# google/deepvariant

Hardware: AMD Instinct MI355X
Metric: candidate pileups/sec (encode+CNN) (higher is better)
Workload: dtype u8 (encoder) / f16 MFMA, f32 accumulate (CNN); 1 GPU; configs[1] shape: synthetic 30x Illumina pileups, WGS 100x221x7, HIP encode + Inception-v3 MFMA on 1 MI355X per rank, random-init weights; parallelism=interval shards x1, all-gather of probs, collective_world_size=1

## Files before the change

deepvariant_amd/csrc/model.hip:

```cpp
#include <algorithm>
#include <map>
#include <atomic>
#include <cmath>
#include <cstdlib>
#include <cstring>
#include <memory>
#include <thread>

#include <hip/hip_fp16.h>

#include "model_graph.h"
#include "model_kernels.h"
#include "block35.h"
#include "mixed3.h"
#include "chain.h"
#include "stem_fused.h"
#include "calib.h"
#include "layer_export.h"

namespace {

static int stem_sub_batch() {
  static const int v = getenv("DV_STEM_SB") ? std::max(1, atoi(getenv("DV_STEM_SB"))) : (1 << 30);
  return v;
// ... 50 lines not shown
  if (mode >= 2) return true;
  return m->blank_conv4_op >= 0 && &op == &m->ops[m->blank_conv4_op];
}

struct Pass {
  dv_model* m;
  int n;
  hipStream_t stream;
  int first, last;
  int shifted_buf, out_example_off;
  size_t images_off;
  std::vector<char> side_pooled;
  _Float16* out_ptr(int buf) const {
    const size_t halfs = static_cast<size_t>(out_example_off) * m->buffers[buf].bytes_per_example() / 2;
    return m->buf_ptr(buf) + (buf == shifted_buf ? halfs : 0);
  }
};

dv::C8Geom c8_geom(const BufferDesc& b) {
  const TensorGeom g = b.geom();
  return dv::C8Geom{g.h, g.w, g.halo, g.hp, g.wp, g.groups};
}


int enqueue_stem_a(const Pass& ps, int oi) {
  const dv_model* m = ps.m;
  const int n = ps.n;
  const Op &op = m->ops[oi], &c2 = m->ops[oi + 1];
  dv::StemAArgs a{};
  a.in = nullptr;
  a.in_ind = &ext_table(m)->images;
  a.in_off = ps.images_off;
  a.w1 = m->w_ptr(op);
  a.w2 = m->w_ptr(c2);
  a.shift1 = m->shift_ptr(op);
  a.shift2 = m->shift_ptr(c2);
  a.out = m->buf_ptr(c2.out_buf);
  a.og = c8_geom(m->buffers[c2.out_buf]);
  a.N = n;
  a.H = op.ih;
  a.W = op.iw;
  a.C = op.cin_real;
  a.OH1 = op.oh;
  a.OW1 = op.ow;
  a.OH2 = c2.oh;
  a.OW2 = c2.ow;
  a.tiles_y = (c2.oh + dv::kStemA_TH - 1) / dv::kStemA_TH;
  a.tiles_x = (c2.ow + dv::kStemA_TW - 1) / dv::kStemA_TW;
  a.total_tiles = n * a.tiles_y * a.tiles_x;
  a.in_bytes = static_cast<unsigned>(static_cast<size_t>(n) * op.ih * op.iw * op.cin_real);
  if (m->blank_on()) {
    a.blank_thr = m->blank_thr(1);
    a.blank_src = static_cast<const _Float16*>(m->d_blank_c2.ptr);
    a.blank_need = m->blank_thr(5);
  }
  TraceScope tr(ps.stream, std::string(m->blank_on() ? "[blank tiles copied] " : "") + "stem_a conv3x3s2 " + std::to_string(op.cin_real) + "->32 + conv3x3 32->32 (fused)",
                2.0 * n * (static_cast<double>(op.oh) * op.ow * op.kh * op.kw * op.cin_real * op.cout +
                           static_cast<double>(c2.oh) * c2.ow * 9 * 32 * 32),
                static_cast<double>(n) * (op.ih * op.iw * op.cin_real + 2.0 * c2.oh * c2.ow * 32));
  dv::ProfileScope prof(dv::kProfConv, ps.stream);
  dv::launch_stem_a(a, m->stem_a_grid, ps.stream);
  return 2;
}

void report_stem_b_profile(dv::StemBArgs a, int grid, hipStream_t stream) {
  const size_t words = static_cast<size_t>(grid) * 16;
  unsigned long long* d = nullptr;
  if (hipMalloc(&d, words * 8) != hipSuccess) return;
  (void)hipMemsetAsync(d, 0, words * 8, stream);
  a.prof = d;
  dv::launch_stem_b(a, grid, stream);
  std::vector<unsigned long long> h(words);
  (void)hipStreamSynchronize(stream);
  (void)hipMemcpy(h.data(), d, words * 8, hipMemcpyDeviceToHost);
  (void)hipFree(d);
  for (int w = 0; w < 2; ++w) {
    double sum[7] = {0, 0, 0, 0, 0, 0, 0};
    for (int b = 0; b < grid; ++b)
      for (int i = 0; i < 7; ++i) sum[i] += static_cast<double>(h[(b * 2 + w) * 8 + i]);
    const double tiles = static_cast<double>(a.total_tiles);
    fprintf(stderr, "[dv-stem-b wave %d] cycles/tile: issue %.0f conv3 %.0f dma-wait %.0f barrierA %.0f pool %.0f "
                    "barrierB %.0f conv1x1+store %.0f\n", w ? 7 : 0, sum[0] / tiles, sum[1] / tiles,
            sum[6] / tiles, sum[2] / tiles, sum[3] / tiles, sum[4] / tiles, sum[5] / tiles);
  }
  std::map<unsigned long long, std::vector<int>> where;
  for (int b = 0; b < grid; ++b) {
    const unsigned long long v = h[(b * 2) * 8 + 7];
    const unsigned hw = static_cast<unsigned>(v), xcc = static_cast<unsigned>(v >> 32);
    where[(static_cast<unsigned long long>(xcc) << 16) | ((hw >> 8) & 0xffu)].push_back(b);
  }
  int pairs = 0, same_parity = 0, apart256 = 0;
  for (const auto& kv : where) {
    if (kv.second.size() != 2) continue;
    ++pairs;
    const unsigned t0 = (static_cast<unsigned>(h[(kv.second[0] * 2) * 8 + 7]) >> 16) & 15u;
    const unsigned t1 = (static_cast<unsigned>(h[(kv.second[1] * 2) * 8 + 7]) >> 16) & 15u;
    same_parity += (t0 & 1u) == (t1 & 1u);
    apart256 += kv.second[1] - kv.second[0] == 256;
  }
  fprintf(stderr, "[dv-stem-b placement] %zu places for %d workgroups; %d pairs, %d with TG slots of EQUAL parity, "
                  "%d pairs are blocks b / b+256\n", where.size(), grid, pairs, same_parity, apart256);
  for (int cls = 0; cls < 2; ++cls) {
    double sum[7] = {0, 0, 0, 0, 0, 0, 0};
    int nb = 0;
    for (int b = 0; b < grid; ++b) {
      const unsigned tg = (static_cast<unsigned>(h[(b * 2) * 8 + 7]) >> 16) & 15u;
      if (static_cast<int>(tg & 1u) != cls) continue;
      ++nb;
      for (int i = 0; i < 7; ++i) sum[i] += static_cast<double>(h[(b * 2) * 8 + i]);
    }
    double tot = 0;
    for (double v : sum) tot += v;
    fprintf(stderr, "[dv-stem-b TG parity %d] %d workgroups, share of wave-0 cycles: issue %.3f conv3 %.3f dma-wait %.3f "
                    "barrierA %.3f pool %.3f barrierB %.3f conv1x1+store %.3f; cycles per workgroup %.0f\n", cls, nb,
            sum[0] / tot, sum[1] / tot, sum[6] / tot, sum[2] / tot, sum[3] / tot, sum[4] / tot, sum[5] / tot,
            nb ? tot / nb : 0.0);
  }
}

int enqueue_stem_b(const Pass& ps, int oi) {
  const dv_model* m = ps.m;
  const int n = ps.n;
  const Op &op = m->ops[oi], &c4 = m->ops[oi + 1];
  const BufferDesc& ib = m->buffers[op.in_buf];
  dv::StemBArgs a{};
  a.in = m->buf_ptr(op.in_buf);
  a.w3 = m->w_ptr(op);
  a.w4 = m->w_ptr(c4);
  a.shift3 = m->shift_ptr(op);
  a.shift4 = m->shift_ptr(c4);
  a.out = m->buf_ptr(c4.out_buf);
  a.ig = c8_geom(ib);
  a.og = c8_geom(m->buffers[c4.out_buf]);
  a.N = n;
  a.OH3 = op.oh;
  a.OW3 = op.ow;
  a.PH = c4.oh;
  a.PW = c4.ow;
  a.Cout4 = c4.cout;
  a.tiles_y = (c4.oh + dv::kStemB_PH - 1) / dv::kStemB_PH;
  a.tiles_x = (c4.ow + dv::kStemB_PW - 1) / dv::kStemB_PW;
  a.total_tiles = n * a.tiles_y * a.tiles_x;
  a.in_bytes = static_cast<size_t>(n) * ib.bytes_per_example();
  a.in_img_bytes = static_cast<unsigned>(ib.bytes_per_example());
  if (m->blank_on()) {
    a.blank_thr = m->blank_thr(2);
    a.blank_src = static_cast<const _Float16*>(m->d_blank_b.ptr);
    a.blank_need = m->blank_thr(6);
  }
  TraceScope tr(ps.stream, std::string(m->blank_on() ? "[blank tiles copied] " : "") + "stem_b conv3x3 32->64 + maxpool3s2 + conv1x1 64->" + std::to_string(c4.cout) + " (fused)",
                2.0 * n * (static_cast<double>(op.oh) * op.ow * 9 * 32 * 64 +
                           static_cast<double>(c4.oh) * c4.ow * 64 * c4.cout),
                2.0 * n * (static_cast<double>(op.ih) * op.iw * 32 + static_cast<double>(c4.oh) * c4.ow * c4.cout));
  dv::ProfileScope prof(dv::kProfConv, ps.stream);
  static const bool stem_prof = getenv("DV_STEM_PROF") != nullptr;
  if (stem_prof && g_trace != nullptr) {
    report_stem_b_profile(a, m->stem_b_grid, ps.stream);
  } else {
    dv::launch_stem_b(a, m->stem_b_grid, ps.stream);
  }
  return 2;
}

int enqueue_block35(const Pass& ps, int oi) {
  const dv_model* m = ps.m;
  const int n = ps.n;
  const Op &op = m->ops[oi], &r5 = m->ops[oi + 1], &r3 = m->ops[oi + 2], &pj = m->ops[oi + 3];
  const Op &c5 = m->ops[oi + 4], &c3a = m->ops[oi + 5], &c3b = m->ops[oi + 6], &ap = m->ops[oi + 7];
  const BufferDesc& ib = m->buffers[op.in_buf];
  dv::Block35Args a{};
  a.in = m->buf_ptr(op.in_buf);
  a.ig = ib.geom();
  a.in_img_bytes = static_cast<unsigned>(ib.bytes_per_example());
  a.N = n;
  a.h = op.oh;
  a.w = op.ow;
  a.n_chunks = op.cin / kChunk;
  a.w1 = m->w_ptr(op);
  a.sh_red5 = m->shift_ptr(r5);
  a.sh_red3 = m->shift_ptr(r3);
  a.sh_b1 = m->shift_ptr(op);
  a.sh_pool = m->shift_ptr(ap);
  a.pool_c = pj.cout;
  a.w5 = m->w_ptr(c5);
  a.sh5 = m->shift_ptr(c5);
  a.w3a = m->w_ptr(c3a);
  a.sh3a = m->shift_ptr(c3a);
  a.w3b = m->w_ptr(c3b);
  a.sh3b = m->shift_ptr(c3b);
  a.out = m->buf_ptr(op.out_buf);
  a.og = m->buffers[op.out_buf].geom();
  a.goff_b1 = op.out_coff / 8;
  a.goff_5 = c5.out_coff / 8;
  a.goff_3 = c3b.out_coff / 8;
  a.goff_pool = ap.out_coff / 8;
  const double px = static_cast<double>(n) * op.oh * op.ow;
  const double tr_flops = 2.0 * px * (static_cast<double>(op.cin) * (op.cout + r5.cout + r3.cout + pj.cout) +
                                      25.0 * c5.cin * c5.cout + 9.0 * c3a.cin * c3a.cout + 9.0 * c3b.cin * c3b.cout);
  const std::string tr_label = "block35 " + std::to_string(op.cin) + "->" + std::to_string(op.cout) + "|" +
                               std::to_string(r5.cout) + "->" + std::to_string(c5.cout) + " 5x5|" +
                               std::to_string(r3.cout) + "->" + std::to_string(c3a.cout) + "->" +
                               std::to_string(c3b.cout) + " 3x3|" + std::to_string(pj.cout) + " pool @" +
                               std::to_string(op.oh) + "x" + std::to_string(op.ow);
// ... 389 lines not shown
    return dv::fail(DV_ERR_INVALID_ARGUMENT,
                    "dv_model_create: unsupported shape (need H,W >= 75, C <= 16, max_batch <= 8192)");
  }
  int n_dev = 0;
  if (hipGetDeviceCount(&n_dev) != hipSuccess || n_dev <= 0) {
    return dv::fail(DV_ERR_NO_DEVICE, "no HIP device: libdvhip has no CPU fallback");
  }
  if (device < 0 || device >= n_dev) {
    return dv::fail(DV_ERR_INVALID_ARGUMENT, "bad device ordinal");
  }
  DV_HIP_CHECK(hipSetDevice(device));
  std::unique_ptr<dv_model> m(new dv_model());
  m->device = device;
  m->desc = *desc;
  m->precise = getenv("DV_PRECISE") != nullptr ? atoi(getenv("DV_PRECISE")) != 0 : desc->channels > 8;
  m->build();
  m->stem_a_grid = dv::stem_a_blocks(device);
  m->stem_b_grid = dv::stem_b_blocks(device);
  m->n_cus = dv::stem_a_blocks(device) / 2;
  for (const Op& op : m->ops) {
    const BufferDesc& ob = m->buffers[op.out_buf];
    const double pieces = static_cast<double>(desc->max_batch) * ob.bytes_per_example() / 16.0;
    const double pixels = static_cast<double>(desc->max_batch) * op.oh * op.ow;
    if (pieces >= 2147483648.0 || pixels >= 67108864.0) {
      return dv::fail(DV_ERR_INVALID_ARGUMENT,
                      "dv_model_create: max_batch too large for this image size (N*OH*OW must stay "
                      "below 2^26 and every activation tensor below 2^31 16-byte pieces)");
    }
  }
  if (static_cast<double>(desc->max_batch) * desc->height * desc->width * desc->channels >=
      2147483648.0) {
    return dv::fail(DV_ERR_INVALID_ARGUMENT, "dv_model_create: max_batch * H * W * C must be < 2^31");
  }
  m->dbuf.resize(m->buffers.size());
  for (size_t i = 0; i < m->buffers.size(); ++i) {
    const BufferDesc& b = m->buffers[i];
    const bool stem_buf = static_cast<int>(i) < m->stem_out_buf;
    const size_t examples = std::max(
        static_cast<size_t>(stem_buf ? std::min(desc->max_batch, stem_sub_batch()) : desc->max_batch),
        static_cast<size_t>(b.min_examples));
    const size_t bytes = examples * b.bytes_per_example() +
                         static_cast<size_t>(8) * (b.h + 2 * b.halo) * (b.w + 2 * b.halo) * 16;
    if (int rc = m->dbuf[i].reserve(bytes)) return rc;
    DV_HIP_CHECK(hipMemset(m->dbuf[i].ptr, 0, m->dbuf[i].cap));
  }
  if (int rc = m->d_w.reserve(m->packed_halfs * 2)) return rc;
  if (int rc = m->d_shift.reserve(m->shift_floats * 4)) return rc;
  if (int rc = m->d_dense_w.reserve(static_cast<size_t>(m->feat_c) * desc->num_classes * 4)) return rc;
  if (int rc = m->d_dense_b.reserve(desc->num_classes * 4)) return rc;
  if (int rc = m->d_ext.reserve(sizeof(ExtPtrs))) return rc;
  if (!(getenv("DV_BLANK_SKIP") != nullptr && atoi(getenv("DV_BLANK_SKIP")) == 0) &&
      m->ops[0].first_u8 && m->blank_conv4_op >= 0 && m->ops[m->blank_conv4_op].group_followers == 0 &&
      (static_cast<size_t>(desc->height) * desc->width * desc->channels) % 4 == 0) {
    if (int rc = m->d_blank_thr.reserve(static_cast<size_t>(7) * desc->max_batch * sizeof(int))) return rc;
    DV_HIP_CHECK(hipMemset(m->d_blank_thr.ptr, 0, m->d_blank_thr.cap));
    m->blank_skip = true;
  }
  *out = m.release();
  return DV_OK;
}

void dv_model_destroy(dv_model* m) {
  if (!m) return;
  (void)hipSetDevice(m->device);
  for (auto& b : m->dbuf) b.release();
  m->d_w.release();
  m->d_shift.release();
  m->d_dense_w.release();
  m->d_dense_b.release();
  m->d_tbl.release();
  m->d_blank_thr.release();
  m->d_ext.release();
  m->d_blank_conv4.release();
  m->d_blank_c2.release();
  m->d_blank_b.release();
  for (auto& g : m->graphs) (void)hipGraphExecDestroy(g.exec);
  delete m;
}

int64_t dv_model_num_params(const dv_model* m) { return m ? m->n_params : 0; }

int64_t dv_model_conv_macs(const dv_model* m) {
  if (!m) return 0;
  int64_t macs = 0;
  for (const Op& op : m->ops) {
    if (op.type == kOpConv) {
      macs += static_cast<int64_t>(op.kh) * op.kw * op.cin_real * op.cout * op.oh * op.ow;
    }
  }
  return macs;
}

int dv_model_num_layers(const dv_model* m) {
  return m ? static_cast<int>(m->layers.size()) : 0;
}

int dv_model_layer_info(const dv_model* m, int layer, int32_t* kh, int32_t* kw,
                        int32_t* cin, int32_t* cout, int64_t* param_offset) {
  if (!m || layer < 0 || layer >= static_cast<int>(m->layers.size())) {
    return dv::fail(DV_ERR_INVALID_ARGUMENT, "dv_model_layer_info: bad layer");
  }
  const LayerInfo& l = m->layers[layer];
  if (kh) *kh = l.kh;
  if (kw) *kw = l.kw;
  if (cin) *cin = l.cin;
  if (cout) *cout = l.cout;
  if (param_offset) *param_offset = l.param_off;
  return DV_OK;
}
// ... 675 lines not shown
```

deepvariant_amd/csrc/model_graph.h:

```cpp
#ifndef DV_MODEL_GRAPH_H_
#define DV_MODEL_GRAPH_H_

#include <string>
#include <vector>

#include "dv_internal.h"
#include "conv_mfma.h"
#include "imgconv.h"

namespace dv {
namespace graph {

using namespace convk;

struct TensorRef {
  int buf = -1;
  int h = 0, w = 0, c = 0;
};

struct BufferDesc {
  int h, w, c;
  int halo = 0;
  int min_examples = 1;
  bool f32 = false;
// ... 28 lines not shown
  bool pool_shift_relu = false;
  bool pool_in = false;
  int side_pool_partner = -1;
  int avg_partner = -1;
  int avg_tile_g = 0;
  bool pool_out = false;
  int band = 0;
  bool split = false;
  bool split_rows = false;
  int split_tiles = 0;
  bool v2 = false;
  int v2_g = 0;
  int v2_steps = 0;
  int v2_tiles = 0;
  bool stem_a = false;
  bool stem_b = false;
  int chain_len = 0;
  int chain_g = 0;
  int chain_tpx = 0;
  bool in_chain = false;
  int b35 = 0;
  int m3 = 0;
};

struct LayerInfo {
  int kh, kw, cin, cout;
  int64_t param_off;
};

}
}

using namespace dv::graph;

struct dv_model {
  int device = 0;
  dv_model_desc desc{};
  std::vector<BufferDesc> buffers;
  std::vector<Op> ops;
  std::vector<LayerInfo> layers;
  int64_t n_params = 0;
  int feat_buf = -1, feat_p = 0, feat_c = 0;
  int stem_ops_end = 0, stem_out_buf = -1;
  int stem_a_grid = 512, stem_b_grid = 256;
  int n_cus = 256;
  size_t packed_halfs = 0, shift_floats = 0, tbl_entries = 0;
  std::vector<dv::DeviceBuffer> dbuf;
  dv::DeviceBuffer d_w, d_shift, d_dense_w, d_dense_b, d_tbl;
  bool blank_skip = false;
  bool blank_enabled = true;
  bool blank_ready = false;
  int blank_conv4_op = -1;
  dv::DeviceBuffer d_blank_thr;
  dv::DeviceBuffer d_blank_conv4;
  dv::DeviceBuffer d_blank_c2;
  dv::DeviceBuffer d_blank_b;
  bool blank_on() const { return blank_ready && blank_enabled; }
  bool precise = false;
  bool wide_stage = false;
  bool loaded = false;
  std::vector<float> h_shift, h_dense_b;
  dv::DeviceBuffer d_ext;
  struct GraphEntry {
    int n;
    hipStream_t stream;
    hipGraphExec_t exec;
  };
  std::vector<GraphEntry> graphs;
  int64_t graph_captures = 0, graph_replays = 0;
  struct NamedView {
    std::string name;
    int buf, coff, c;
  };
  std::vector<NamedView> named_views;

  template <typename T = _Float16>
  T* buf_ptr(int buf) const { return static_cast<T*>(dbuf[buf].ptr); }
  const _Float16* w_ptr(const Op& op) const { return static_cast<const _Float16*>(d_w.ptr) + op.w_off; }
  const float* shift_ptr(const Op& op) const { return static_cast<const float*>(d_shift.ptr) + op.shift_off; }
  const int* blank_thr(int row) const { return static_cast<const int*>(d_blank_thr.ptr) + row * desc.max_batch; }

  int new_buffer(int h, int w, int c);
  static int pick_nb(int cout);
  TensorRef conv(TensorRef x, int cout, int kh, int kw, int stride = 1, bool same = true,
                 int dst_buf = -1, int dst_coff = 0, int cin_real = -1);
  TensorRef full(int buf) const;
  void pooled_projection(TensorRef x, int cout, int dst_buf, int dst_coff);
  TensorRef pool(OpType type, TensorRef x, int dst_buf = -1, int dst_coff = 0);
  void group_siblings();
  dv::ImgConvArgs imgconv_geometry(const Op& op, int g) const;
  void choose_imgconv();
  void choose_band();
  void choose_side_pool();
  void choose_split();
  void choose_avg_epilogue();
  void choose_chains();
  void choose_block35();
  void choose_mixed3();
  void build();
  std::vector<size_t> correction_shift_offsets() const;
};

#endif
```

deepvariant_amd/csrc/model_kernels.hip:

```cpp
#include <cstdlib>

#include "model_kernels.h"
#include "stem_fused.h"

using namespace dv::convk;

namespace {

constexpr int kFirstUnroll = 5;

__global__ void set_ext_kernel(ExtPtrs* ext, const uint8_t* images, float* probs, const int32_t* rows_hint, int rows_add) {
  ext->images = images;
  ext->probs = probs;
  ext->rows_hint = rows_hint;
  ext->rows_add = rows_add;
}

__device__ __forceinline__ const uint8_t* ext_images(const ExtPtrs* ext, size_t off) {
  const unsigned long long v = reinterpret_cast<unsigned long long>(ext->images + off);
  const unsigned lo = __builtin_amdgcn_readfirstlane(static_cast<unsigned>(v));
  const unsigned up = __builtin_amdgcn_readfirstlane(static_cast<unsigned>(v >> 32));
  return reinterpret_cast<const uint8_t*>((static_cast<unsigned long long>(up) << 32) | lo);
}

// ... 114 lines not shown
                             co + 2 * hq + 1 < p.Cout ? p.shift[co + 2 * hq + 1] : 0.f};
        const float2_t v = float2_t{acc[pt][4 * q + 2 * hq], acc[pt][4 * q + 2 * hq + 1]} + sv;
        half2_t h = __builtin_convertvector(v, half2_t);
        h = __builtin_elementwise_max(h, zero2);
        pk[q][hq] = __builtin_bit_cast(unsigned, h);
      }
    }
#pragma unroll
    for (int t2 = 0; t2 < 2; ++t2) {
      const auto d0 = __builtin_amdgcn_permlane32_swap(pk[2 * t2][0], pk[2 * t2 + 1][0], false, false);
      const auto d1 = __builtin_amdgcn_permlane32_swap(pk[2 * t2][1], pk[2 * t2 + 1][1], false, false);
      const uint4_t piece = {d0[0], d1[0], d0[1], d1[1]};
      const int group = 2 * t2 + hi;
      if (mvalid[pt] && group * 8 < p.Cout) {
        outp[obase[pt] + static_cast<unsigned>(group) * gstride] = piece;
      }
    }
  }
}

__global__ void preprocess_kernel(const ExtPtrs* ext, size_t in_off, _Float16* out, size_t n_pix, int C,
                                  int H, int W, TensorGeom og) {
  const size_t i = blockIdx.x * static_cast<size_t>(blockDim.x) + threadIdx.x;
  if (i >= n_pix) return;
  const uint8_t* in = ext->images + in_off;
  const uint8_t* px = in + i * C;
  _Float16 v[16];
#pragma unroll
  for (int c = 0; c < 16; ++c) {
    v[c] = c < C ? static_cast<_Float16>((static_cast<float>(px[c]) - 128.0f) / 128.0f)
                 : static_cast<_Float16>(0.f);
  }
  const size_t n = i / (static_cast<size_t>(H) * W);
  const int pix = static_cast<int>(i - n * (static_cast<size_t>(H) * W));
  const int y = pix / W, x = pix - y * W;
  uint4* dst = reinterpret_cast<uint4*>(out);
  const size_t plane = static_cast<size_t>(og.hp) * og.wp;
  const size_t at = (n * 2) * plane + static_cast<size_t>(y + og.halo) * og.wp + x + og.halo;
  dst[at] = *reinterpret_cast<uint4*>(&v[0]);
  dst[at + plane] = *reinterpret_cast<uint4*>(&v[8]);
}

__global__ void blank_need_kernel(int* thr, int stride, int n, int oh2, int ph_b, int ow4, int p4, int stem_b_fused,
                                  int conv4_walks) {
  const int i = blockIdx.x * blockDim.x + threadIdx.x;
  if (i >= n) return;
  const int t4 = min(thr[2 * stride + i], ph_b);
  const int kb = (t4 + dv::kStemB_PH - 1) / dv::kStemB_PH;
  thr[5 * stride + i] = !stem_b_fused ? oh2 : kb > 0 ? min(oh2, 2 * dv::kStemB_PH * kb + 2) : 0;
  const int span = 31 / max(ow4, 1) + 1;
  int m5 = 0;
  for (int j = max(0, i - span); j <= min(n - 1, i + span); ++j) m5 = max(m5, min(thr[4 * stride + j], p4));
  thr[6 * stride + i] = !conv4_walks ? ph_b : m5 > 0 ? min(ph_b, 2 * m5 + 3) : 0;
}

__global__ __launch_bounds__(256) void blank_rows_kernel(const ExtPtrs* ext, size_t in_off, int n_hint0, int H,
                                                         int row_bytes, int* thr, int stride) {
  __shared__ int last;
  const uint8_t* images = ext->images + in_off;
  const int n = blockIdx.x, tid = threadIdx.x;
  const unsigned img_bytes = static_cast<unsigned>(H) * row_bytes;
  const uint32_t* img = reinterpret_cast<const uint32_t*>(images + static_cast<size_t>(n) * img_bytes);
  const int n_dw = static_cast<int>(img_bytes / 4);
  if (tid == 0) last = -1;
  __syncthreads();
  constexpr int kPer = 16;
  const bool hinted = ext->rows_hint != nullptr;
  const int hinted_rows = hinted ? max(0, min(H, ext->rows_hint[n_hint0 + n] + ext->rows_add)) : 0;
  for (int hi = hinted ? 0 : n_dw; hi > 0; hi -= 256 * kPer) {
    uint32_t v[kPer];
#pragma unroll
    for (int k = 0; k < kPer; ++k) {
      const int i = hi - 1 - (k * 256 + tid);
      v[k] = i >= 0 ? img[i] : 0u;
    }
    int mine = -1;
#pragma unroll
    for (int k = 0; k < kPer; ++k) {
      const int i = hi - 1 - (k * 256 + tid);
      if (v[k] != 0) mine = max(mine, 4 * i + 3 - (__clz(v[k]) >> 3));
    }
    if (mine >= 0) atomicMax(&last, mine);
    __syncthreads();
    if (last >= 0) break;
  }
  if (tid == 0) {
    const int r = hinted ? hinted_rows : last < 0 ? 0 : last / row_bytes + 1;
    const int t2 = (r + 1) / 2, t3 = t2 + 1, t4 = (t3 + 1) / 2;
    thr[n] = r;
    thr[stride + n] = t2;
    thr[2 * stride + n] = t4;
    thr[3 * stride + n] = t4;
    thr[4 * stride + n] = (t4 + 1) / 2;
  }
}

__global__ void maxpool3s2_kernel(PoolArgs p) {
  const int cg = p.C / 8;
  const size_t total = static_cast<size_t>(p.N) * cg * p.OH * p.OW;
  const size_t i = blockIdx.x * static_cast<size_t>(blockDim.x) + threadIdx.x;
  if (i >= total) return;
  const int ow = i % p.OW;
  size_t t = i / p.OW;
  const int oh = t % p.OH;
  t /= p.OH;
  const int g = t % cg;
  const int n = t / cg;
  const size_t plane = static_cast<size_t>(p.ig.hp) * p.ig.wp;
  const half8_t* src = reinterpret_cast<const half8_t*>(p.in) + (static_cast<size_t>(n) * p.ig.groups + g) * plane;
  const half8_t* src_lo = src + static_cast<size_t>(p.lo_in_groups) * plane;
  half8_t best, best_lo;
#pragma unroll
  for (int j = 0; j < 8; ++j) {
    best[j] = static_cast<_Float16>(-65504.f);
    best_lo[j] = static_cast<_Float16>(0.f);
  }
  const size_t at0 = static_cast<size_t>(oh * 2 + p.ig.halo) * p.ig.wp + ow * 2 + p.ig.halo;
  if (p.lo_in_groups > 0) {
    half8_t v[9], l[9];
#pragma unroll
    for (int t9 = 0; t9 < 9; ++t9) {
      const size_t at = at0 + static_cast<size_t>(t9 / 3) * p.ig.wp + t9 % 3;
      v[t9] = src[at];
      l[t9] = src_lo[at];
    }
#pragma unroll
    for (int t9 = 0; t9 < 9; ++t9) {
#pragma unroll
      for (int j = 0; j < 8; ++j) {
        const bool take = v[t9][j] > best[j] || (v[t9][j] == best[j] && l[t9][j] > best_lo[j]);
        best[j] = take ? v[t9][j] : best[j];
        best_lo[j] = take ? l[t9][j] : best_lo[j];
      }
    }
  } else {
    for (int dh = 0; dh < 3; ++dh)
      for (int dw = 0; dw < 3; ++dw) {
// ... 207 lines not shown
```

deepvariant_amd/csrc/stem.hip:

```cpp
#include <algorithm>
#include <type_traits>

#include "stem_fused.h"

namespace dv {
namespace {

typedef _Float16 half8_t __attribute__((ext_vector_type(8)));
typedef _Float16 half2_t __attribute__((ext_vector_type(2)));
typedef float float16_t __attribute__((ext_vector_type(16)));
typedef float float4_t __attribute__((ext_vector_type(4)));
typedef float float2_t __attribute__((ext_vector_type(2)));
typedef unsigned uint4_t __attribute__((ext_vector_type(4)));
typedef unsigned uint3_t __attribute__((ext_vector_type(3)));

__device__ __forceinline__ half8_t lds_piece(const char* smem, unsigned off) {
  return *reinterpret_cast<const half8_t*>(smem + off);
}

__device__ __forceinline__ float16_t acc_init(const float* tbl) {
  const float4_t* t = reinterpret_cast<const float4_t*>(tbl);
  const float4_t a = t[0], b = t[1], c = t[2], d = t[3];
  return float16_t{a[0], a[1], a[2], a[3], b[0], b[1], b[2], b[3],
                   c[0], c[1], c[2], c[3], d[0], d[1], d[2], d[3]};
// ... 210 lines not shown
    }
  };

  auto convert_patch = [&](unsigned org) {
#pragma unroll
    for (int ps = 0; ps < A_PASSES; ++ps) {
      if (sact && (ps * A_ROWS_PER_PASS + srow < A_INH)) {
        const unsigned a = org + srel + ps * spass;
        const unsigned s8 = (a & 3u) * 8u;
        const unsigned lo = __builtin_amdgcn_alignbit(pre[ps][1], pre[ps][0], s8);
        const unsigned up = __builtin_amdgcn_alignbit(pre[ps][2], pre[ps][1], s8);
        if constexpr (WIDE) {
          typedef unsigned uint2_t __attribute__((ext_vector_type(2)));
          const unsigned lo1 = __builtin_amdgcn_alignbit(pre[ps][3], pre[ps][2], s8);
          char* d = smem + sdst + ps * (A_ROWS_PER_PASS * AW_ROW);
          *reinterpret_cast<uint2_t*>(d) = uint2_t{lo, up};
          *reinterpret_cast<uint2_t*>(d + AW_PLANE) = uint2_t{lo1, 0u};
        } else {
          *reinterpret_cast<uint4_t*>(smem + sdst + ps * (A_ROWS_PER_PASS * A_INROW)) =
              normalise8(lo, up);
        }
      }
    }
  };
  auto copy_blank_tile = [&](int nb_, int yb, int xb) {
    const uint4_t* src = reinterpret_cast<const uint4_t*>(p.blank_src);
    uint4_t* dst = reinterpret_cast<uint4_t*>(p.out) + static_cast<size_t>(nb_) * img_out;
    const int th = min(A_TH, p.OH2 - yb), tw = min(A_TW, p.OW2 - xb);
    const int per_group = th * tw;
    constexpr int kPer = (4 * A_TH * A_TW + A_THREADS - 1) / A_THREADS;
    uint4_t v[kPer];
    unsigned at[kPer];
#pragma unroll
    for (int k = 0; k < kPer; ++k) {
      const int e = k * A_THREADS + tid;
      const int g = e / per_group, r = e - g * per_group;
      const int yy = r / tw, xx = r - yy * tw;
      at[k] = e < 4 * per_group ? static_cast<unsigned>(g) * gstride +
                                      static_cast<unsigned>((yb + yy + p.og.halo) * p.og.wp + xb + xx + p.og.halo)
                                : 0xffffffffu;
      if (at[k] != 0xffffffffu) v[k] = src[at[k]];
    }
#pragma unroll
    for (int k = 0; k < kPer; ++k) {
      if (at[k] != 0xffffffffu) dst[at[k]] = v[k];
    }
  };
  auto next_tile = [&](int tt) {
    if (p.blank_thr == nullptr) return tt;
    while (tt < p.total_tiles) {
      int nb_, yb, xb;
      tile_origin(tt, nb_, yb, xb);
      if (yb < p.blank_thr[nb_]) break;
      if (yb < p.blank_need[nb_]) copy_blank_tile(nb_, yb, xb);
      tt += gridDim.x;
    }
    return tt;
  };
  int t = next_tile(blockIdx.x);
  int n, y0, x0;
  unsigned origin = 0;
  if (t < p.total_tiles) {
    origin = tile_origin(t, n, y0, x0);
    issue_loads(origin);
    convert_patch(origin);
  }
  while (t < p.total_tiles) {
    __syncthreads();

#pragma unroll
    for (int round = 0; round < 2; ++round) {
      float16_t acc[2];
#pragma unroll
      for (int f = 0; f < 2; ++f) acc[f] = acc_init(lsh + hi * 16);
      if constexpr (WIDE) {
        typedef unsigned uint2_t __attribute__((ext_vector_type(2)));
        auto b_addr = [&](int tap, int f) {
          const int kh = tap / 3, kw = tap % 3;
          return bA[round * 2 + f] + static_cast<unsigned>((kw & 1) * 2 * AW_PLANE + kh * AW_ROW + (kw >> 1) * 8);
        };
        const char* w1l = smem + AW_OFF_W1 + (hi * 32 + l31) * 16;
        half8_t wa[2];
        uint2_t xb[2][2];
        wa[0] = lds_piece(w1l, 0);
#pragma unroll
        for (int f = 0; f < 2; ++f) xb[0][f] = *reinterpret_cast<const uint2_t*>(smem + b_addr(0, f));
#pragma unroll
        for (int tap = 0; tap < 9; ++tap) {
          if (tap + 1 < 9) {
            wa[(tap + 1) & 1] = lds_piece(w1l, (tap + 1) * 2 * 32 * 16);
#pragma unroll
            for (int f = 0; f < 2; ++f) xb[(tap + 1) & 1][f] = *reinterpret_cast<const uint2_t*>(smem + b_addr(tap + 1, f));
          }
#pragma unroll
          for (int f = 0; f < 2; ++f) {
            const half8_t x = __builtin_bit_cast(half8_t, normalise8(xb[tap & 1][f][0], xb[tap & 1][f][1]));
            acc[f] = __builtin_amdgcn_mfma_f32_32x32x16_f16(wa[tap & 1], x, acc[f], 0, 0, 0);
          }
        }
      } else
      mfma_sweep<5, 2, 3>(
          a1, smem,
          [&](int s, int f) {
            const int ff = round * 2 + f;
            return s < 3 ? bA[ff] + s * A_INROW : s == 3 ? bB[ff] + 16 : bC[ff] + 2 * A_INROW + 16;
          },
          acc);
// ... 56 lines not shown
constexpr int B_PTH = B_C3H + 2, B_PTW = B_C3W + 2;
constexpr int B_PTPX = B_PTH * B_PTW;
constexpr int B_PTPLANE = B_PTPX * 16;
constexpr int B_PT_BYTES = (4 * B_PTPLANE + 1023) / 1024 * 1024;
constexpr int B_PT_PIECES = 4 * B_PTPX;
constexpr int B_PPX = B_PH * B_PW;
constexpr int B_PFR = (B_PPX + 31) / 32;
constexpr int B_PPLANE = B_PFR * 32 * 16;
constexpr int B_THREADS = B_WAVES * 64;
constexpr int B_PASSES = (B_PT_PIECES + B_THREADS - 1) / B_THREADS;
constexpr int B_POOL_ROUNDS = (8 * B_PPX + B_THREADS - 1) / B_THREADS;
constexpr int B_OFF_C3 = 2 * B_PT_BYTES;
constexpr int B_OFF_P = (B_OFF_C3 + 8 * B_C3PLANE + 15) / 16 * 16;
constexpr int B_OFF_SH = B_OFF_P + 8 * B_PPLANE;
constexpr int B_LDS = B_OFF_SH + (64 + 96) * 4;
constexpr int B_BLOCKS_PER_CU = B_WAVES == 4 ? 2 : 1;
static_assert(B_LDS * B_BLOCKS_PER_CU <= 160 * 1024, "workgroups per CU");
static_assert(2 * B_PFR == B_WAVES, "1x1 work split: (pooled fragment, subtiles {0,1}) and (fragment, subtile 2)");
static_assert(B_C3FR <= 2 * B_WAVES, "two conv3 fragments per wave");

__global__ __launch_bounds__(B_THREADS, 2) void stem_b_kernel(StemBArgs p) {
  extern __shared__ __attribute__((aligned(16))) char smem[];
  const int tid = threadIdx.x;
  const int lane = tid & 63, wave = tid >> 6;
  const int hi = lane >> 5, l31 = lane & 31;
  const int wave_u = __builtin_amdgcn_readfirstlane(wave);

  half8_t a3lo[18], a3up[18];
#pragma unroll
  for (int kc = 0; kc < 18; ++kc) {
    a3lo[kc] = *reinterpret_cast<const half8_t*>(p.w3 + (((0 * 18 + kc) * 2 + hi) * 32 + l31) * 8);
    a3up[kc] = *reinterpret_cast<const half8_t*>(p.w3 + (((1 * 18 + kc) * 2 + hi) * 32 + l31) * 8);
  }
  const int s0 = wave < B_PFR ? 0 : 2;
  const int nsub = wave < B_PFR ? 2 : 1;
#pragma unroll
  for (int kc = 0; kc < 18; ++kc) {
    asm volatile("" : "+v"(a3lo[kc]));
    asm volatile("" : "+v"(a3up[kc]));
  }
  float* lsh = reinterpret_cast<float*>(smem + B_OFF_SH);
  if (tid < 160) {
    const int r = tid & 15, h = (tid >> 4) & 1;
    const int co = (r & 3) + 8 * (r >> 2) + 4 * h;
    if (tid < 64) {
      lsh[tid] = p.shift3[(tid >> 5) * 32 + co];
    } else {
      const int c4 = ((tid - 64) >> 5) * 32 + co;
      lsh[tid] = c4 < p.Cout4 ? p.shift4[c4] : 0.f;
    }
  }

  unsigned prel[B_PASSES];
#pragma unroll
  for (int ps = 0; ps < B_PASSES; ++ps) {
    const int e = ps * B_THREADS + tid;
    const int g = e / B_PTPX, rem = e - g * B_PTPX;
    const int row = rem / B_PTW, col = rem - row * B_PTW;
    prel[ps] = e < B_PT_PIECES
                   ? static_cast<unsigned>(((g * p.ig.hp + row) * p.ig.wp + col) * 16)
                   : 0x80000000u;
  }
  unsigned b3[2], c3dst[2];
  bool c3ok[2];
#pragma unroll
  for (int m = 0; m < 2; ++m) {
    const int i = (wave + B_WAVES * m) * 32 + l31;
    c3ok[m] = i < B_C3PX;
    const int ii = min(i, B_C3PX - 1);
    const int cy = ii / B_C3W, cx = ii - cy * B_C3W;
    b3[m] = static_cast<unsigned>(hi * B_PTPLANE + (cy * B_PTW + cx) * 16);
    c3dst[m] = static_cast<unsigned>(B_OFF_C3 + hi * B_C3PLANE + i * 16);
  }
  const int pp = (wave % B_PFR) * 32 + l31;
  const int ppc = min(pp, B_PPX - 1);
  const int ppy = ppc / B_PW, ppx = ppc - ppy * B_PW;
  const unsigned b4 = static_cast<unsigned>(B_OFF_P + hi * B_PPLANE + pp * 16);

  const int tiles_img = p.tiles_y * p.tiles_x;
  const unsigned ogstride = static_cast<unsigned>(p.og.hp * p.og.wp);

  auto tile_coords = [&](int t, int& n, int& py0, int& px0) {
    n = t / tiles_img;
    const int r = t - n * tiles_img;
    const int ty = r / p.tiles_x;
    py0 = ty * B_PH;
    px0 = (r - ty * p.tiles_x) * B_PW;
  };
  auto patch_desc = [&](int n) {
    const size_t off = static_cast<size_t>(n) * p.in_img_bytes;
    const size_t left = p.in_bytes - off;
    const unsigned long long base = reinterpret_cast<unsigned long long>(p.in) + off;
    const unsigned blo = __builtin_amdgcn_readfirstlane(static_cast<unsigned>(base));
    const unsigned bup = __builtin_amdgcn_readfirstlane(static_cast<unsigned>(base >> 32));
    return __builtin_amdgcn_make_buffer_rsrc(
        reinterpret_cast<char*>((static_cast<unsigned long long>(bup) << 32) | blo), 0,
        static_cast<unsigned>(left < 0x7fffffffu ? left : 0x7fffffffu), 0x00020000);
  };
  auto patch_soff = [&](int py0, int px0) {
    return static_cast<unsigned>(((2 * py0 - 1 + p.ig.halo) * p.ig.wp + 2 * px0 - 1 + p.ig.halo) * 16);
  };
  auto dma_round = [&](int ps, const __amdgpu_buffer_rsrc_t rsrc, unsigned soff, unsigned buf_off) {
    const unsigned g0 = static_cast<unsigned>((ps * B_WAVES + wave_u) * 1024);
    if (g0 < static_cast<unsigned>(B_PT_BYTES)) {
      __builtin_amdgcn_raw_ptr_buffer_load_lds(
          rsrc, (__attribute__((address_space(3))) void*)(smem + buf_off + g0), 16, prel[ps], soff, 0, 0);
    }
  };

  auto copy_blank_tile = [&](int nb_, int pyb, int pxb) {
    const uint4_t* src = reinterpret_cast<const uint4_t*>(p.blank_src);
    uint4_t* dst = reinterpret_cast<uint4_t*>(p.out) +
                   static_cast<size_t>(nb_) * p.og.groups * ogstride;
    const int th = min(B_PH, p.PH - pyb), tw = min(B_PW, p.PW - pxb);
    const int per_group = th * tw;
    const int groups = (p.Cout4 + 7) / 8;
    constexpr int kPer = (12 * B_PH * B_PW + B_THREADS - 1) / B_THREADS;
    uint4_t v[kPer];
    unsigned at[kPer];
#pragma unroll
    for (int k = 0; k < kPer; ++k) {
      const int e = k * B_THREADS + tid;
      const int g = e / per_group, r = e - g * per_group;
      const int yy = r / tw, xx = r - yy * tw;
      at[k] = e < groups * per_group ? static_cast<unsigned>(g) * ogstride +
                                           static_cast<unsigned>((pyb + yy + p.og.halo) * p.og.wp + pxb + xx + p.og.halo)
                                     : 0xffffffffu;
      if (at[k] != 0xffffffffu) v[k] = src[at[k]];
    }
#pragma unroll
    for (int k = 0; k < kPer; ++k) {
      if (at[k] != 0xffffffffu) dst[at[k]] = v[k];
    }
  };
  auto next_tile = [&](int tt) {
    if (p.blank_thr == nullptr) return tt;
    while (tt < p.total_tiles) {
      int nb_, pyb, pxb;
      tile_coords(tt, nb_, pyb, pxb);
      if (pyb < p.blank_thr[nb_]) break;
      if (pyb < p.blank_need[nb_]) copy_blank_tile(nb_, pyb, pxb);
      tt += gridDim.x;
    }
    return tt;
  };
  int t = next_tile(blockIdx.x);
  int n = 0, py0 = 0, px0 = 0;
  unsigned buf = 0;
  if (t < p.total_tiles) {
    tile_coords(t, n, py0, px0);
    const __amdgpu_buffer_rsrc_t r0 = patch_desc(n);
    const unsigned so0 = patch_soff(py0, px0);
#pragma unroll
    for (int ps = 0; ps < B_PASSES; ++ps) dma_round(ps, r0, so0, 0);
  }
  asm volatile("s_waitcnt vmcnt(0) lgkmcnt(0)\n\ts_barrier" ::: "memory");
  unsigned long long ph[7] = {0, 0, 0, 0, 0, 0, 0};
  unsigned long long tm = p.prof ? __builtin_amdgcn_s_memtime() : 0;
#define DV_PHASE(i_)                                          \
  if (p.prof) {                                               \
    const unsigned long long now_ = __builtin_amdgcn_s_memtime(); \
    ph[i_] += now_ - tm;                                      \
    tm = now_;                                                \
  }
  while (t < p.total_tiles) {
    const int tn = next_tile(t + gridDim.x);
    int nn = 0, pyn = 0, pxn = 0;
    const bool more = tn < p.total_tiles;
    if (more) tile_coords(tn, nn, pyn, pxn);
    const __amdgpu_buffer_rsrc_t rn = patch_desc(more ? nn : n);
    const unsigned son = patch_soff(pyn, pxn);
    DV_PHASE(0)

#pragma unroll
    for (int m = 0; m < 2; ++m) {
      if (wave + B_WAVES * m < B_C3FR) {
        float16_t acc_lo = acc_init(lsh + hi * 16), acc_up = acc_init(lsh + 32 + hi * 16);
        mfma_sweep_pair<18, 4>(
            a3lo, a3up, smem,
            [&](int s) {
              const int tap = s >> 1, c = s & 1;
              return buf + b3[m] + c * 2 * B_PTPLANE + ((tap / 3) * B_PTW + tap % 3) * 16;
            },
            acc_lo, acc_up,
            [&](int sI) {
              if (m == 0 && more && sI % 3 == 0 && sI / 3 < B_PASSES) {
                dma_round(sI / 3, rn, son, buf ^ B_PT_BYTES);
              }
            });
        if (c3ok[m]) {
          *reinterpret_cast<uint4_t*>(smem + c3dst[m]) = relu_piece(acc_lo, 0);
          *reinterpret_cast<uint4_t*>(smem + c3dst[m] + 2 * B_C3PLANE) = relu_piece(acc_lo, 1);
          *reinterpret_cast<uint4_t*>(smem + c3dst[m] + 4 * B_C3PLANE) = relu_piece(acc_up, 0);
          *reinterpret_cast<uint4_t*>(smem + c3dst[m] + 6 * B_C3PLANE) = relu_piece(acc_up, 1);
        }
      }
    }
    half8_t a4[8];
#pragma unroll
    for (int sI = 0; sI < 2; ++sI) {
      const int sub = min(s0 + sI, 2);
#pragma unroll
      for (int c = 0; c < 4; ++c) {
        a4[sI * 4 + c] = *reinterpret_cast<const half8_t*>(p.w4 + (((sub * 4 + c) * 2 + hi) * 32 + l31) * 8);
      }
    }
    DV_PHASE(1)
    if (p.prof) {
      asm volatile("s_waitcnt vmcnt(0)" ::: "memory");
      DV_PHASE(6)
    }
    asm volatile("s_waitcnt vmcnt(0) lgkmcnt(0)\n\ts_barrier" ::: "memory");
    DV_PHASE(2)

#pragma unroll
    for (int k = 0; k < B_POOL_ROUNDS; ++k) {
      const int e = k * B_THREADS + tid;
      if (e < 8 * B_PPX) {
        const int j = e >> 1;
        const int q = 2 * (j / B_PPX) + (e & 1), pq = j % B_PPX;
        const int qy = pq / B_PW, qx = pq - qy * B_PW;
        const char* src = smem + B_OFF_C3 + q * B_C3PLANE + (2 * qy * B_C3W + 2 * qx) * 16;
        half8_t win[9];
#pragma unroll
        for (int w9 = 0; w9 < 9; ++w9) {
          win[w9] = *reinterpret_cast<const half8_t*>(src + ((w9 / 3) * B_C3W + w9 % 3) * 16);
        }
        __builtin_amdgcn_sched_barrier(0);
        const half8_t m01 = __builtin_elementwise_max(win[0], win[1]);
        const half8_t m23 = __builtin_elementwise_max(win[2], win[3]);
        const half8_t m45 = __builtin_elementwise_max(win[4], win[5]);
        const half8_t m67 = __builtin_elementwise_max(win[6], win[7]);
        const half8_t best = __builtin_elementwise_max(
            __builtin_elementwise_max(__builtin_elementwise_max(m01, m23), __builtin_elementwise_max(m45, m67)),
            win[8]);
        *reinterpret_cast<half8_t*>(smem + B_OFF_P + q * B_PPLANE + pq * 16) = best;
      }
    }
    DV_PHASE(3)
    __syncthreads();
// ... 179 lines not shown
```

deepvariant_amd/csrc/stem_fused.h:

```cpp
#ifndef DV_STEM_FUSED_H_
#define DV_STEM_FUSED_H_

#include <hip/hip_runtime.h>

#include <cstddef>
#include <cstdint>

namespace dv {

struct C8Geom {
  int h, w, halo, hp, wp, groups;
};

constexpr int kStemA_TH = 7, kStemA_TW = 54;
constexpr int kStemA_W1Halfs = 5 * 2 * 32 * 8;
constexpr int kStemA_W2Halfs = 18 * 2 * 32 * 8;
constexpr int kStemA_W1WideHalfs = 9 * 2 * 32 * 8;
constexpr int kStemA_MaxChannels = 12;

struct StemAArgs {
  const uint8_t* in;
  const uint8_t* const* in_ind;
  size_t in_off;
  const _Float16* w1;
  const _Float16* w2;
  const float* shift1;
  const float* shift2;
  _Float16* out;
  C8Geom og;
  int N, H, W, C;
  int OH1, OW1, OH2, OW2;
  int tiles_y, tiles_x;
  int total_tiles;
  unsigned in_bytes;
  const int* blank_thr;
  const _Float16* blank_src;
  const int* blank_need;
};

#ifdef DV_STEM_B_WIDE
constexpr int kStemB_PH = 12, kStemB_PW = 9, kStemB_Waves = 8;
#else
constexpr int kStemB_PH = 6, kStemB_PW = 9, kStemB_Waves = 4;
#endif
constexpr int kStemB_W3Halfs = 2 * 18 * 2 * 32 * 8;
constexpr int kStemB_W4Halfs = 3 * 4 * 2 * 32 * 8;

struct StemBArgs {
  const _Float16* in;
  const _Float16* w3;
  const _Float16* w4;
  const float* shift3;
  const float* shift4;
  _Float16* out;
  C8Geom ig, og;
  int N;
  int OH3, OW3;
  int PH, PW;
  int Cout4;
  int tiles_y, tiles_x;
  int total_tiles;
  size_t in_bytes;
  unsigned in_img_bytes;
  unsigned long long* prof;
  const int* blank_thr;
  const _Float16* blank_src;
  const int* blank_need;
};

void launch_stem_a(const StemAArgs& a, int blocks, hipStream_t stream);
void launch_stem_b(const StemBArgs& a, int blocks, hipStream_t stream);
int stem_a_blocks(int device);
int stem_b_blocks(int device);

void pack_stem_a_w1(const float* w, const float* inv, int cin, _Float16* dst);
void pack_stem_a_w1_wide(const float* w, const float* inv, int cin, _Float16* dst);
void pack_stem_a_w2(const float* w, const float* inv, _Float16* dst);
void pack_stem_b_w3(const float* w, const float* inv, _Float16* dst);
void pack_stem_b_w4(const float* w, const float* inv, int cout, _Float16* dst);

}

#endif
```

Baseline: 512,300 candidates/s.

## Let stem_b read blank rows from a precomputed blank image instead of stem_a copying tiles

Stem_a no longer copies precomputed blank tiles into its output. Instead stem_b's patch DMA switches, per row, to a buffer descriptor pointing at a precomputed blank stem_a output for rows past a new per-example cut threshold (a new eighth row of the threshold table). Stem_b also replaces per-tile blank copies with a single per-row strip copy issued by the first tile column. This removes redundant blank-tile writes and reads in the stem, at the cost of a per-load branch, an extra buffer descriptor, and more register and control complexity. The blank_rows kernel also gets an extra barrier to fix a race on the shared 'last' value.

```diff
diff --git a/deepvariant_amd/csrc/model.hip b/deepvariant_amd/csrc/model.hip
--- a/deepvariant_amd/csrc/model.hip
+++ b/deepvariant_amd/csrc/model.hip
@@ -126,9 +126,9 @@
   if (m->blank_on()) {
     a.blank_thr = m->blank_thr(1);
     a.blank_src = static_cast<const _Float16*>(m->d_blank_c2.ptr);
-    a.blank_need = m->blank_thr(5);
-  }
-  TraceScope tr(ps.stream, std::string(m->blank_on() ? "[blank tiles copied] " : "") + "stem_a conv3x3s2 " + std::to_string(op.cin_real) + "->32 + conv3x3 32->32 (fused)",
+    a.blank_need = m->blank_read_through() ? nullptr : m->blank_thr(5);
+  }
+  TraceScope tr(ps.stream, std::string(!m->blank_on() ? "" : m->blank_read_through() ? "[blank tiles left to stem_b] " : "[blank tiles copied] ") + "stem_a conv3x3s2 " + std::to_string(op.cin_real) + "->32 + conv3x3 32->32 (fused)",
                 2.0 * n * (static_cast<double>(op.oh) * op.ow * op.kh * op.kw * op.cin_real * op.cout +
                            static_cast<double>(c2.oh) * c2.ow * 9 * 32 * 32),
                 static_cast<double>(n) * (op.ih * op.iw * op.cin_real + 2.0 * c2.oh * c2.ow * 32));
@@ -221,8 +221,13 @@
     a.blank_thr = m->blank_thr(2);
     a.blank_src = static_cast<const _Float16*>(m->d_blank_b.ptr);
     a.blank_need = m->blank_thr(6);
-  }
-  TraceScope tr(ps.stream, std::string(m->blank_on() ? "[blank tiles copied] " : "") + "stem_b conv3x3 32->64 + maxpool3s2 + conv1x1 64->" + std::to_string(c4.cout) + " (fused)",
+    a.blank_strip = m->blank_copy_tiles ? 0 : 1;
+    if (m->blank_read_through()) {
+      a.blank_cut = m->blank_thr(7);
+      a.blank_in = static_cast<const _Float16*>(m->d_blank_c2.ptr);
+    }
+  }
+  TraceScope tr(ps.stream, std::string(!m->blank_on() ? "" : m->blank_copy_tiles ? "[blank tiles copied] " : m->blank_read_through() ? "[blank rows read through, blank strip copied] " : "[blank strip copied] ") + "stem_b conv3x3 32->64 + maxpool3s2 + conv1x1 64->" + std::to_string(c4.cout) + " (fused)",
                 2.0 * n * (static_cast<double>(op.oh) * op.ow * 9 * 32 * 64 +
                            static_cast<double>(c4.oh) * c4.ow * 64 * c4.cout),
                 2.0 * n * (static_cast<double>(op.ih) * op.iw * 32 + static_cast<double>(c4.oh) * c4.ow * c4.cout));
@@ -718,9 +723,10 @@
   if (!(getenv("DV_BLANK_SKIP") != nullptr && atoi(getenv("DV_BLANK_SKIP")) == 0) &&
       m->ops[0].first_u8 && m->blank_conv4_op >= 0 && m->ops[m->blank_conv4_op].group_followers == 0 &&
       (static_cast<size_t>(desc->height) * desc->width * desc->channels) % 4 == 0) {
-    if (int rc = m->d_blank_thr.reserve(static_cast<size_t>(7) * desc->max_batch * sizeof(int))) return rc;
+    if (int rc = m->d_blank_thr.reserve(static_cast<size_t>(dv_model::kBlankThrRows) * desc->max_batch * sizeof(int))) return rc;
     DV_HIP_CHECK(hipMemset(m->d_blank_thr.ptr, 0, m->d_blank_thr.cap));
     m->blank_skip = true;
+    m->blank_copy_tiles = getenv("DV_BLANK_COPY_TILES") != nullptr && atoi(getenv("DV_BLANK_COPY_TILES")) != 0;
   }
   *out = m.release();
   return DV_OK;
diff --git a/deepvariant_amd/csrc/model_graph.h b/deepvariant_amd/csrc/model_graph.h
--- a/deepvariant_amd/csrc/model_graph.h
+++ b/deepvariant_amd/csrc/model_graph.h
@@ -104,10 +104,15 @@
   bool blank_ready = false;
   int blank_conv4_op = -1;
   dv::DeviceBuffer d_blank_thr;
+  static constexpr int kBlankThrRows = 8;
   dv::DeviceBuffer d_blank_conv4;
   dv::DeviceBuffer d_blank_c2;
   dv::DeviceBuffer d_blank_b;
   bool blank_on() const { return blank_ready && blank_enabled; }
+  bool blank_copy_tiles = false;
+  bool blank_read_through() const {
+    return blank_on() && !blank_copy_tiles && ops.size() > 3 && ops[0].stem_a && ops[2].stem_b && d_blank_c2.ptr != nullptr;
+  }
   bool precise = false;
   bool wide_stage = false;
   bool loaded = false;
diff --git a/deepvariant_amd/csrc/model_kernels.hip b/deepvariant_amd/csrc/model_kernels.hip
--- a/deepvariant_amd/csrc/model_kernels.hip
+++ b/deepvariant_amd/csrc/model_kernels.hip
@@ -190,6 +190,8 @@
   int m5 = 0;
   for (int j = max(0, i - span); j <= min(n - 1, i + span); ++j) m5 = max(m5, min(thr[4 * stride + j], p4));
   thr[6 * stride + i] = !conv4_walks ? ph_b : m5 > 0 ? min(ph_b, 2 * m5 + 3) : 0;
+  const int t2 = max(thr[stride + i], 0);
+  thr[7 * stride + i] = min(oh2, dv::kStemA_TH * ((t2 + dv::kStemA_TH - 1) / dv::kStemA_TH));
 }
 
 __global__ __launch_bounds__(256) void blank_rows_kernel(const ExtPtrs* ext, size_t in_off, int n_hint0, int H,
@@ -220,7 +222,9 @@
     }
     if (mine >= 0) atomicMax(&last, mine);
     __syncthreads();
-    if (last >= 0) break;
+    const int found = last;
+    __syncthreads();
+    if (found >= 0) break;
   }
   if (tid == 0) {
     const int r = hinted ? hinted_rows : last < 0 ? 0 : last / row_bytes + 1;
diff --git a/deepvariant_amd/csrc/stem.hip b/deepvariant_amd/csrc/stem.hip
--- a/deepvariant_amd/csrc/stem.hip
+++ b/deepvariant_amd/csrc/stem.hip
@@ -286,7 +286,7 @@
       int nb_, yb, xb;
       tile_origin(tt, nb_, yb, xb);
       if (yb < p.blank_thr[nb_]) break;
-      if (yb < p.blank_need[nb_]) copy_blank_tile(nb_, yb, xb);
+      if (p.blank_need != nullptr && yb < p.blank_need[nb_]) copy_blank_tile(nb_, yb, xb);
       tt += gridDim.x;
     }
     return tt;
@@ -449,6 +449,8 @@
   }
 
   unsigned prel[B_PASSES];
+  unsigned prow = 0;
+  static_assert(B_PTH <= 64 && 6 * B_PASSES <= 32, "the patch rows of all passes pack into one register");
 #pragma unroll
   for (int ps = 0; ps < B_PASSES; ++ps) {
     const int e = ps * B_THREADS + tid;
@@ -457,6 +459,7 @@
     prel[ps] = e < B_PT_PIECES
                    ? static_cast<unsigned>(((g * p.ig.hp + row) * p.ig.wp + col) * 16)
                    : 0x80000000u;
+    prow |= (e < B_PT_PIECES ? static_cast<unsigned>(row) : 0u) << (6 * ps);
   }
   unsigned b3[2], c3dst[2];
   bool c3ok[2];
@@ -497,11 +500,23 @@
   auto patch_soff = [&](int py0, int px0) {
     return static_cast<unsigned>(((2 * py0 - 1 + p.ig.halo) * p.ig.wp + 2 * px0 - 1 + p.ig.halo) * 16);
   };
-  auto dma_round = [&](int ps, const __amdgpu_buffer_rsrc_t rsrc, unsigned soff, unsigned buf_off) {
+  const __amdgpu_buffer_rsrc_t rblank = __builtin_amdgcn_make_buffer_rsrc(
+      const_cast<_Float16*>(p.blank_cut != nullptr ? p.blank_in : p.in), 0, p.in_img_bytes, 0x00020000);
+  auto patch_rcut = [&](int n, int py0) {
+    return p.blank_cut != nullptr ? p.blank_cut[n] - (2 * py0 - 1) : 0x7fffffff;
+  };
+  auto dma_round = [&](int ps, const __amdgpu_buffer_rsrc_t rsrc, unsigned soff, unsigned buf_off, int rcut) {
     const unsigned g0 = static_cast<unsigned>((ps * B_WAVES + wave_u) * 1024);
     if (g0 < static_cast<unsigned>(B_PT_BYTES)) {
-      __builtin_amdgcn_raw_ptr_buffer_load_lds(
-          rsrc, (__attribute__((address_space(3))) void*)(smem + buf_off + g0), 16, prel[ps], soff, 0, 0);
+      auto* dst = (__attribute__((address_space(3))) void*)(smem + buf_off + g0);
+      unsigned rows = prow;
+      asm volatile("" : "+v"(rows));
+      if (static_cast<int>((rows >> (6 * ps)) & 63u) < rcut) {
+        __builtin_amdgcn_raw_ptr_buffer_load_lds(rsrc, dst, 16, prel[ps], soff, 0, 0);
+      } else {
+        __builtin_amdgcn_raw_ptr_buffer_load_lds(rblank, dst, 16, prel[ps], soff, 0, 0);
+        asm volatile("");
+      }
     }
   };
 
@@ -530,13 +545,45 @@
       if (at[k] != 0xffffffffu) dst[at[k]] = v[k];
     }
   };
+  auto copy_blank_strip = [&](int nb_, int row0, int row1) {
+    const uint4_t* src = reinterpret_cast<const uint4_t*>(p.blank_src);
+    uint4_t* dst = reinterpret_cast<uint4_t*>(p.out) +
+                   static_cast<size_t>(nb_) * p.og.groups * ogstride;
+    const int per_group = (row1 - row0) * p.PW;
+    const int total = (p.Cout4 + 7) / 8 * per_group;
+    constexpr int kPer = 3;
+    for (int e0 = 0; e0 < total; e0 += kPer * B_THREADS) {
+      uint4_t v[kPer];
+      unsigned at[kPer];
+#pragma unroll
+      for (int k = 0; k < kPer; ++k) {
+        const int e = e0 + k * B_THREADS + tid;
+        const int g = e / per_group, r = e - g * per_group;
+        const int yy = r / p.PW, xx = r - yy * p.PW;
+        at[k] = e < total ? static_cast<unsigned>(g) * ogstride +
+                                static_cast<unsigned>((row0 + yy + p.og.halo) * p.og.wp + xx + p.og.halo)
+                          : 0xffffffffu;
+        if (at[k] != 0xffffffffu) v[k] = src[at[k]];
+      }
+#pragma unroll
+      for (int k = 0; k < kPer; ++k) {
+        if (at[k] != 0xffffffffu) dst[at[k]] = v[k];
+      }
+    }
+  };
   auto next_tile = [&](int tt) {
     if (p.blank_thr == nullptr) return tt;
     while (tt < p.total_tiles) {
       int nb_, pyb, pxb;
       tile_coords(tt, nb_, pyb, pxb);
-      if (pyb < p.blank_thr[nb_]) break;
-      if (pyb < p.blank_need[nb_]) copy_blank_tile(nb_, pyb, pxb);
+      const int thr = p.blank_thr[nb_];
+      if (pyb < thr) break;
+      const int need = p.blank_need[nb_];
+      if (p.blank_strip) {
+        if (pxb == 0 && pyb < thr + B_PH && pyb < need) copy_blank_strip(nb_, pyb, need);
+      } else if (pyb < need) {
+        copy_blank_tile(nb_, pyb, pxb);
+      }
       tt += gridDim.x;
     }
     return tt;
@@ -548,8 +595,9 @@
     tile_coords(t, n, py0, px0);
     const __amdgpu_buffer_rsrc_t r0 = patch_desc(n);
     const unsigned so0 = patch_soff(py0, px0);
-#pragma unroll
-    for (int ps = 0; ps < B_PASSES; ++ps) dma_round(ps, r0, so0, 0);
+    const int rc0 = patch_rcut(n, py0);
+#pragma unroll
+    for (int ps = 0; ps < B_PASSES; ++ps) dma_round(ps, r0, so0, 0, rc0);
   }
   asm volatile("s_waitcnt vmcnt(0) lgkmcnt(0)\n\ts_barrier" ::: "memory");
   unsigned long long ph[7] = {0, 0, 0, 0, 0, 0, 0};
@@ -567,6 +615,7 @@
     if (more) tile_coords(tn, nn, pyn, pxn);
     const __amdgpu_buffer_rsrc_t rn = patch_desc(more ? nn : n);
     const unsigned son = patch_soff(pyn, pxn);
+    const int rcn = patch_rcut(more ? nn : n, pyn);
     DV_PHASE(0)
 
 #pragma unroll
@@ -582,7 +631,7 @@
             acc_lo, acc_up,
             [&](int sI) {
               if (m == 0 && more && sI % 3 == 0 && sI / 3 < B_PASSES) {
-                dma_round(sI / 3, rn, son, buf ^ B_PT_BYTES);
+                dma_round(sI / 3, rn, son, buf ^ B_PT_BYTES, rcn);
               }
             });
         if (c3ok[m]) {
diff --git a/deepvariant_amd/csrc/stem_fused.h b/deepvariant_amd/csrc/stem_fused.h
--- a/deepvariant_amd/csrc/stem_fused.h
+++ b/deepvariant_amd/csrc/stem_fused.h
@@ -66,6 +66,9 @@
   const int* blank_thr;
   const _Float16* blank_src;
   const int* blank_need;
+  const int* blank_cut;
+  const _Float16* blank_in;
+  int blank_strip;
 };
 
 void launch_stem_a(const StemAArgs& a, int blocks, hipStream_t stream);
```

Result: faster. 518,800 candidates/s (median of 6 runs) (+1.3%).
